# chaiyujin/sdfa-2019

Hardware: AMD Instinct MI355X
Metric: animation frames/s/node (10 s@16 kHz clips); max|Δdgrad| vs CPU ref (higher is better)
Workload: dtype f32

## Files before the change

sdfa-2019_amd/csrc/api_core.cpp:

```cpp
#include "../../include/sdfa_stream.h"
#include "host.h"

#include <climits>
#include <cstdio>
#include <cstring>
#include <string>

static thread_local std::string g_err;

int sdfa_failv(int code, const char *fmt, va_list ap) {
    char buf[512];
    vsnprintf(buf, sizeof buf, fmt, ap);
    g_err = buf;
    return code;
}

int sdfa_fail(int code, const char *fmt, ...) {
    va_list ap;
    va_start(ap, fmt);
    sdfa_failv(code, fmt, ap);
    va_end(ap);
    return code;
}

thread_local int g_sdfa_mel_fft_radix4 = 0;
thread_local int g_sdfa_gather_plain_order = 0;
thread_local int g_sdfa_frontend_two_kernel = 0;
thread_local int g_sdfa_frontend_stream_block = 0;
thread_local int g_sdfa_frontend_stream_slots = 0;
thread_local int g_sdfa_frontend_stream_spin_max = 0;
thread_local int g_sdfa_frontend_stream_phases = 0;
thread_local int g_sdfa_frontend_t_major = 0;
extern thread_local int g_sdfa_gemm_variant;
thread_local int g_sdfa_freq_lstm_shape = 0;
thread_local int g_sdfa_pca_lds = 0;
thread_local int g_sdfa_pca_fp32 = 0;
thread_local int g_sdfa_conv_fp32 = 0;
thread_local int g_sdfa_time_lstm_split = 0;
thread_local int g_sdfa_time_lstm_handoff = 0;
thread_local int g_sdfa_time_lstm_timeout_us = 0;
thread_local int g_sdfa_share_gx0_off = 0;
thread_local int g_sdfa_encoder_dedup_off = 0;
thread_local int g_sdfa_share_hash_bits = 0;
thread_local int g_sdfa_freq_proj_tail = 0;
thread_local int g_sdfa_attn_unfused = 0;

extern "C" {

int sdfa_abi_version(void) { return SDFA_ABI_VERSION; }
int sdfa_stream_abi_version(void) { return SDFA_STREAM_ABI_VERSION; }
const char *sdfa_last_error(void) { return g_err.c_str(); }

int sdfa_debug_set_option(const char *name, int value) {
    struct Option { const char *name; int *var; int lo = INT_MIN, hi = INT_MAX; const char *accepts = nullptr; };
    thread_local const Option options[] = {
        {"attn_unfused", &g_sdfa_attn_unfused},
        {"share_gx0_off", &g_sdfa_share_gx0_off},
        {"encoder_dedup_off", &g_sdfa_encoder_dedup_off},
        {"share_hash_bits", &g_sdfa_share_hash_bits, 0, 32, "0 (the whole hash) or 1..32 low bits"},
        {"freq_proj_tail", &g_sdfa_freq_proj_tail, 0, 2, "0 (rule), 1 (never) or 2 (always)"},
        {"frontend_two_kernel", &g_sdfa_frontend_two_kernel},
        {"frontend_stream_phases", &g_sdfa_frontend_stream_phases},
        {"frontend_stream_spin_max", &g_sdfa_frontend_stream_spin_max, 0, INT_MAX, "0 (default) or a positive poll count"},
        {"frontend_stream_block", &g_sdfa_frontend_stream_block, 0, 256, "0 (default) or 1..256 frames"},
        {"frontend_stream_slots", &g_sdfa_frontend_stream_slots, 0, 256, "0 (default) or 1..256 workgroups per block"},
        {"gather_plain_order", &g_sdfa_gather_plain_order},
        {"mel_fft_radix4", &g_sdfa_mel_fft_radix4},
        {"frontend_t_major", &g_sdfa_frontend_t_major},
        {"time_lstm_timeout_us", &g_sdfa_time_lstm_timeout_us},
        {"time_lstm_handoff", &g_sdfa_time_lstm_handoff},
        {"time_lstm_split", &g_sdfa_time_lstm_split},
        {"gemm_variant", &g_sdfa_gemm_variant},
        {"freq_lstm_shape", &g_sdfa_freq_lstm_shape},
        {"pca_lds", &g_sdfa_pca_lds},
        {"conv_fp32", &g_sdfa_conv_fp32},
        {"pca_fp32", &g_sdfa_pca_fp32},
    };
    for (const Option &o : options)
        if (name && !strcmp(name, o.name)) {
            if (value < o.lo || value > o.hi) return sdfa_fail(SDFA_EINVAL, "%s: %s", o.name, o.accepts);
            *o.var = value;
            return SDFA_OK;
        }
    return sdfa_fail(SDFA_EINVAL, "unknown option '%s'", name ? name : "(null)");
}

}
```

sdfa-2019_amd/csrc/api_forward.cpp:

```cpp
#include "common.h"
#include "host.h"
#include "kernels.h"
#include "model.h"

#include <algorithm>

extern thread_local int g_sdfa_gemm_variant, g_sdfa_freq_lstm_shape, g_sdfa_pca_lds, g_sdfa_pca_fp32, g_sdfa_conv_fp32, g_sdfa_share_gx0_off, g_sdfa_attn_unfused, g_sdfa_encoder_dedup_off,
    g_sdfa_freq_proj_tail, g_sdfa_share_hash_bits;

namespace {

constexpr int64_t CT_WORDS = 2048, CT_FLAGS = 16, ST_WORDS = SDFA_WS_STATUS_BYTES / 4;

struct Ws {
    int64_t P1, X3, HF, Z, GX, H0, H1, KP, QC, QP, ZK, SH, ZU, total;
    int64_t TRUNK, A0, A1, COEF;
    int64_t CT_FREQ, CT_PCA, CT_FLAG;
};

Ws layout(int64_t Nc, bool keep) {
    const int64_t Mc = 64 * Nc;
    Ws w{};
    int64_t o = 0;
    auto take = [&](int64_t n) { int64_t r = o; o += round_up(n, 64); return r; };
// ... 172 lines not shown
                sa.group_key = sa.hash + Mc; sa.group_first = reinterpret_cast<uint32_t *>(sa.group_key + sa.group_slots);
                sa.hash_bits = g_sdfa_share_hash_bits;
                HIP_TRY(sdfa_launch_share_map_content(sa, s));
            }
            pf.end();
            d_ulimit = sa.counts + 1; d_qfull = sa.counts + 2; col_to_u = sa.col_to_u;
            ca.col_src = sa.col_src; ca.col_limit = d_ulimit;
        }
        const int conv_terms = g_sdfa_conv_fp32 ? 0 : stage_terms(m, STAGE_BODY);
        if (m->keep && conv_terms) {
            pf.begin("conv1"); HIP_TRY(sdfa_launch_conv1(ca, s)); pf.end();
            ca.wb = m->cv_wb; ca.terms = conv_terms;
            pf.begin("conv23"); HIP_TRY(sdfa_launch_conv123(ca, s)); pf.end();
        } else if (m->keep) {
            pf.begin("conv1"); HIP_TRY(sdfa_launch_conv1(ca, s)); pf.end();
            pf.begin("conv23"); HIP_TRY(sdfa_launch_conv23(ca, s)); pf.end();
        } else {
            ca.wb = m->cv_wb; ca.terms = conv_terms;
            pf.begin("conv23"); HIP_TRY(sdfa_launch_conv123(ca, s)); pf.end();
        }

        const int fl_terms = stage_terms(m, STAGE_BODY);
        FreqLstmArgs fa{ws + w.X3, m->fl_w, m->fl_b, ws + w.HF, Mc, d_ulimit, m->fl_wb, fl_terms, reinterpret_cast<int *>(ws + w.CT_FREQ),
                        g_sdfa_freq_lstm_shape ? g_sdfa_freq_lstm_shape : (fl_terms ? 0 : m->freq_shape.load()), m->reserved_cus.load()};
        pf.begin("freq_lstm"); HIP_TRY(sdfa_launch_freq_lstm(fa, s)); pf.end();

        GemmArgs g = sdfa_gemm_k4(m->fp_w, 256, ws + w.HF, Mc, ws + w.Z, Mc, 8192);
        g.bias = m->fp_b; g.q_tile_major = 1; g.q_slab_rows = HF_SLAB_ROWS;
        g.terms = stage_terms(m, STAGE_BODY);
        g.reserve_cus = m->reserved_cus.load();
        if (share) { g.D = ws + w.ZU; g.q_limit = split_tail ? d_qfull : d_ulimit; }
        pf.begin("freq_proj");
        HIP_TRY(sdfa_launch_gemm(g, s));
        if (split_tail) {
            GemmTailArgs gt{m->fp_w, ws + w.HF, m->fp_b, ws + w.ZU, Mc, HF_SLAB_ROWS, d_qfull, d_ulimit, (int)fat_grid - 1};
            HIP_TRY(sdfa_launch_gemm_tail(gt, s));
        }
        pf.end();
        const bool share_gx0 = share && !m->keep && stage_terms(m, STAGE_BODY) == 0 && !g_sdfa_share_gx0_off;
        if (share && !share_gx0) {
            pf.begin("share_expand"); HIP_TRY(sdfa_launch_expand_cols(ws + w.ZU, col_to_u, ws + w.Z, 64, Mc, s)); pf.end();
        }

        const float *xin = share_gx0 ? ws + w.ZU : ws + w.Z;
        float *hout[2] = {ws + w.H0, ws + w.H1};
        const char *gxn[2] = {"gx0", "gx1"}, *lsn[2] = {"lstm0", "lstm1"};
        for (int l = 0; l < 2; ++l) {
            const bool mapped = share_gx0 && l == 0;
            float *gx = mapped ? ws + w.HF : ws + w.GX;
            GemmArgs gi = sdfa_gemm_k4(m->gx_w[l], 2048, xin, Mc, gx, Mc, l == 0 ? 256 : 512);
            gi.terms = stage_terms(m, STAGE_BODY);
            gi.reserve_cus = m->reserved_cus.load();
            if (mapped) gi.q_limit = d_ulimit;
            pf.begin(gxn[l]); HIP_TRY(sdfa_launch_gemm(gi, s)); pf.end();
            TimeLstmArgs ta{gx, m->tl_w[l], hout[l], Nc, Mc, m->tl_wb[l], stage_terms(m, STAGE_BODY),
                            reinterpret_cast<unsigned *>(ws + w.CT_FLAG), CT_WORDS - CT_FLAGS, m->tl_w16[l],
                            reinterpret_cast<unsigned *>(ws), m->reserved_cus.load(), mapped ? col_to_u : nullptr};
            pf.begin(lsn[l]); HIP_TRY(sdfa_launch_time_lstm(ta, s)); pf.end();
            xin = hout[l];
        }
        const int at_terms = stage_terms(m, STAGE_ATTENTION);
        const bool key_fused = g_sdfa_attn_unfused != 1;
        pf.begin("attn_proj");
        GemmArgs gk = sdfa_gemm_k4(m->kp_w, 128, ws + w.H1, Mc, ws + w.KP, Mc, 512);
        gk.terms = at_terms;
        if (!key_fused) HIP_TRY(sdfa_launch_gemm(gk, s));
        GemmArgs gc = sdfa_gemm_k4(m->qc_w, 512, ws + w.H1 + 31 * Nc * 4, Mc, ws + w.QC, Nc, 1536);
        gc.seg_k = 512; gc.seg_col = Nc; gc.terms = at_terms;
        HIP_TRY(sdfa_launch_gemm(gc, s));
        GemmArgs gq = sdfa_gemm_k4(m->qp_w, 128, ws + w.QC, Nc, ws + w.QP, Nc, 512);
        gq.terms = at_terms;
        HIP_TRY(sdfa_launch_gemm(gq, s));
        const bool tail_fused = key_fused && (at_terms == 0 || at_terms == 6) && g_sdfa_attn_unfused != 2 && sdfa_attn_fuses_tail(Nc, m->reserved_cus.load());
        if (key_fused) {
            AttnKeyArgs ak{};
            ak.Wk = m->kp_w; ak.H = ws + w.H1; ak.QP = ws + w.QP; ak.v = m->at_v; ak.b = m->at_b;
            ak.S = ws + w.KP;
            ak.Nc = Nc; ak.Mc = Mc; ak.terms = at_terms == 6 ? 0 : at_terms; ak.reserve_cus = m->reserved_cus.load();
            if (tail_fused) {
                ak.fuse_tail = 1; ak.Zk4 = ws + w.ZK; ak.z_out = d_z + f0 * 512; ak.align_out = d_align ? d_align + f0 * 64 : nullptr; ak.N = N;
            }
            HIP_TRY(sdfa_launch_attn_key_score(ak, s));
        }
        pf.end();

        AttnArgs aa{};
        aa.KP = ws + w.KP; aa.QP = ws + w.QP; aa.H = ws + w.H1; aa.v = m->at_v; aa.b = m->at_b;
        aa.Zk4 = ws + w.ZK; aa.z_out = d_z + f0 * 512; aa.align_out = d_align ? d_align + f0 * 64 : nullptr;
        aa.N = N; aa.Nc = Nc; aa.Mc = Mc;
        aa.S = key_fused ? ws + w.KP : nullptr;
        pf.begin("attn"); if (!tail_fused) HIP_TRY(sdfa_launch_attn(aa, s)); pf.end();
    }
    return SDFA_OK;
}

int sdfa_model_autotune(sdfa_model *m, int64_t n_frames, void *d_workspace, int64_t workspace_bytes, void *stream) {
    if (!m || !m->finalized) return sdfa_fail(SDFA_ESTATE, "autotune: model not finalised");
    if (!d_workspace || n_frames <= 0 || ((uintptr_t)d_workspace & 15)) return sdfa_fail(SDFA_EINVAL, "autotune: bad argument");
    const int64_t cap = capacity(workspace_bytes, m->keep);
    if (cap < 128) return sdfa_fail(SDFA_ENOSPACE, "autotune: workspace too small");
    const int64_t Nc = round_up(std::min(cap, n_frames), 128), Mc = 64 * Nc;
    const Ws w = layout(Nc, m->keep);
    float *ws = (float *)d_workspace;
    hipStream_t s = (hipStream_t)stream;
    HIP_TRY(hipMemsetAsync(ws + w.X3, 0, (size_t)2048 * Mc * sizeof(float), s));
    hipEvent_t e0, e1;
    HIP_TRY(hipEventCreate(&e0));
    HIP_TRY(hipEventCreate(&e1));
    static const int forms[] = {9, 8, 5, 3};
    float best_ms = 0.f;
// ... 204 lines not shown
```

sdfa-2019_amd/csrc/api_model.cpp:

```cpp
#include "host.h"
#include "kernels.h"
#include "model.h"

#include <cmath>
#include <cstring>

namespace {

const std::vector<float> *get(const sdfa_model *m, const std::string &name, size_t numel) {
    auto it = m->host.find(name);
    if (it == m->host.end()) { sdfa_fail(SDFA_ESTATE, "tensor '%s' missing", name.c_str()); return nullptr; }
    if (it->second.size() != numel) {
        sdfa_fail(SDFA_ESTATE, "tensor '%s' has %zu elements, expected %zu", name.c_str(), it->second.size(), numel);
        return nullptr;
    }
    return &it->second;
}

struct Packer {
    std::vector<float> buf;
    struct Bind { const float **f; const void **v; size_t o; };
    std::vector<Bind> binds;
    size_t add(size_t n) {
        size_t o = (buf.size() + 63) / 64 * 64;
// ... 244 lines not shown
        const auto perm = gate_perm(128);
        const char *suf[2] = {"", "_reverse"};
        std::vector<float> cat((size_t)512 * 192);
        size_t first = 0;
        std::vector<float> bias(1024);
        auto gate_scale = [](int torch_row) { return torch_row / 128 == 2 ? TWO_LOG2E : LOG2E; };
        for (int d = 0; d < 2; ++d) {
            const std::string k = enc + "6._lstm.";
            auto *wih = get(m, k + "weight_ih_l0" + suf[d], 512 * 64), *whh = get(m, k + "weight_hh_l0" + suf[d], 512 * 128);
            auto *bih = get(m, k + "bias_ih_l0" + suf[d], 512), *bhh = get(m, k + "bias_hh_l0" + suf[d], 512);
            if (!wih || !whh || !bih || !bhh) return SDFA_ESTATE;
            for (int r = 0; r < 512; ++r) {
                const float k = gate_scale(r);
                for (int j = 0; j < 64; ++j) cat[(size_t)r * 192 + j] = (*wih)[(size_t)r * 64 + j] * k;
                for (int j = 0; j < 128; ++j) cat[(size_t)r * 192 + 64 + j] = (*whh)[(size_t)r * 128 + j] * k;
            }
            size_t o = pack_k4(pk, cat.data(), 512, 192, 192, 0, 192, 512, perm.data());
            pack_freq_lstm_bf16(reinterpret_cast<uint16_t *>(&pk.buf[o_flwb]) + (size_t)d * 3 * 24 * 512 * 8, cat.data(), perm.data());
            if (d == 0) first = pk.bind(m->fl_w, o);
            else if (o != first + (size_t)48 * 512 * 4) return sdfa_fail(SDFA_ESTATE, "internal: freq-lstm weights not contiguous");
            for (int p = 0; p < 512; ++p)
                bias[d * 512 + p] = ((*bih)[perm[p]] + (*bhh)[perm[p]]) * gate_scale(perm[p]);
        }
        memcpy(&pk.buf[pk.bind(m->fl_b, pk.add(1024))], bias.data(), 1024 * 4);
    }
    {
        auto *w = get(m, enc + "6._proj.weight", (size_t)256 * 8192), *b = get(m, enc + "6._proj.bias", 256);
        if (!w || !b) return SDFA_ESTATE;
        pk.bind(m->fp_w, pack_k4(pk, w->data(), 256, 8192, 8192, 0, 8192, 256));
        memcpy(&pk.buf[pk.bind(m->fp_b, pk.add(256))], b->data(), 256 * 4);
    }
    {
        size_t o_tlb[2], o_tl16[2];
        const auto perm = gate_perm(256);
        for (int l = 0; l < 2; ++l) o_tlb[l] = pk.bind(m->tl_wb[l], pk.add((size_t)2 * 3 * 32 * 1024 * 8 / 2));
        for (int l = 0; l < 2; ++l) o_tl16[l] = pk.bind(m->tl_w16[l], pk.add((size_t)2 * 16 * 4 * 1024 * 4));
        const char *suf[2] = {"", "_reverse"};
        for (int l = 0; l < 2; ++l) {
            const int Kin = l == 0 ? 256 : 512;
            std::vector<float> both((size_t)2048 * Kin);
            size_t first = 0;
            for (int d = 0; d < 2; ++d) {
                auto *wih = get(m, enc + "9.weight_ih_l" + std::to_string(l) + suf[d], (size_t)1024 * Kin);
                auto *whh = get(m, enc + "9.weight_hh_l" + std::to_string(l) + suf[d], (size_t)1024 * 256);
                if (!wih || !whh) return SDFA_ESTATE;
                for (int p = 0; p < 1024; ++p) memcpy(&both[((size_t)d * 1024 + p) * Kin], &(*wih)[(size_t)perm[p] * Kin], Kin * 4);
                size_t o = pack_k4(pk, whh->data(), 1024, 256, 256, 0, 256, 1024, perm.data());
                pack_rec_bf16(reinterpret_cast<uint16_t *>(&pk.buf[o_tlb[l]]) + (size_t)d * 3 * 32 * 1024 * 8, whh->data(), perm.data());
                pack_rec_16x16x4(&pk.buf[o_tl16[l]] + (size_t)d * 16 * 4 * 1024 * 4, whh->data(), perm.data());
                if (d == 0) first = pk.bind(m->tl_w[l], o);
                else if (o != first + (size_t)64 * 1024 * 4) return sdfa_fail(SDFA_ESTATE, "internal: time-lstm weights not contiguous");
            }
            pk.bind(m->gx_w[l], pack_k4(pk, both.data(), 2048, Kin, Kin, 0, Kin, 2048));
        }
    }
    {
        const std::string k = enc + "10.";
        auto *cq = get(m, k + "_conv_query.weight", (size_t)512 * 512 * 3), *wk = get(m, k + "proj_key.weight", 128 * 512);
        auto *wq = get(m, k + "proj_qry.weight", 128 * 512), *v = get(m, k + "v.weight", 128), *b = get(m, k + "b", 128);
        if (!cq || !wk || !wq || !v || !b) return SDFA_ESTATE;
        pk.bind(m->kp_w, pack_k4(pk, wk->data(), 128, 512, 512, 0, 512, 128));
        pk.bind(m->qp_w, pack_k4(pk, wq->data(), 128, 512, 512, 0, 512, 128));
        std::vector<float> flat((size_t)512 * 1536);
        for (int o = 0; o < 512; ++o)
            for (int c = 0; c < 512; ++c)
                for (int t = 0; t < 3; ++t) flat[(size_t)o * 1536 + t * 512 + c] = (*cq)[((size_t)o * 512 + c) * 3 + t];
        pk.bind(m->qc_w, pack_k4(pk, flat.data(), 512, 1536, 1536, 0, 1536, 512));
        memcpy(&pk.buf[pk.bind(m->at_v, pk.add(128))], v->data(), 512);
        memcpy(&pk.buf[pk.bind(m->at_b, pk.add(128))], b->data(), 512);
    }
    const std::string om = "_output_module.";
    auto pack_basis = [&](int b, const std::vector<float> &compT, int kreal, const std::vector<float> &means) {
        pk.bind(m->pca_q[b], pack_k4(pk, compT.data(), (int)m->pca_cols[b], kreal, kreal, 0, m->pca_K[b], (int)m->pca_ld[b]));
        memcpy(&pk.buf[pk.bind(m->pca_bias[b], pk.add(m->pca_ld[b]))], means.data(), m->pca_cols[b] * 4);
    };
    if (m->head == SDFA_HEAD_DGRAD) {
        if (pack_fc(m, pk, om + "_layers.0", 512, 512, true, ACT_LRELU, m->trunk)) return SDFA_ESTATE;
        const char *brn[2] = {"_scale_layers.", "_rotat_layers."};
        const int nco[2] = {SDFA_COEF_SCALE, SDFA_COEF_ROTAT};
        for (int b = 0; b < 2; ++b) {
            if (pack_fc(m, pk, om + brn[b] + "0", 512, 512, true, ACT_LRELU, m->br[b][0])) return SDFA_ESTATE;
            if (pack_fc(m, pk, om + brn[b] + "1", 256, 512, false, ACT_TANH, m->br[b][1])) return SDFA_ESTATE;
            if (pack_fc(m, pk, om + brn[b] + "2", nco[b], 256, false, ACT_NONE, m->br[b][2])) return SDFA_ESTATE;
        }
        auto *cs = get(m, om + "_scale_pca.compT", (size_t)59856 * 85), *ms = get(m, om + "_scale_pca.means", 59856);
        auto *cr = get(m, om + "_rotat_pca.compT", (size_t)29928 * 180), *mr = get(m, om + "_rotat_pca.means", 29928);
        if (!cs || !ms || !cr || !mr) return SDFA_ESTATE;
        m->pca_n = 2;
        const std::vector<float> *comp[2] = {cs, cr}, *mean[2] = {ms, mr};
        const int kreal[2] = {85, 180};
        for (int b = 0; b < 2; ++b) {
            m->pca_K[b] = b ? 192 : 96; m->pca_k0[b] = b ? 96 : 0; m->pca_group[b] = b ? 3 : 6; m->pca_off[b] = b ? 6 : 0;
            m->pca_cols[b] = b ? 29928 : 59856; m->pca_ld[b] = round_up(m->pca_cols[b], 128);
            pack_basis(b, *comp[b], kreal[b], *mean[b]);
        }
        {
            const int64_t ntb = (m->pca_cols[1] + 95) / 96;
            const size_t o_pqb = pk.bind(m->pca_qb, pk.add((size_t)ntb * 2 * (12 * 192 + 24 * 96) * 8 / 2));
            pack_pca_bf16(reinterpret_cast<uint16_t *>(&pk.buf[o_pqb]), cs->data(), cr->data(), m->pca_cols[0], m->pca_cols[1], ntb);
        }
    } else {
        if (pack_fc(m, pk, om + "_layers.0", 512, 512, true, ACT_LRELU, m->off[0])) return SDFA_ESTATE;
        if (pack_fc(m, pk, om + "_layers.1", 256, 512, false, ACT_TANH, m->off[1])) return SDFA_ESTATE;
        if (pack_fc(m, pk, om + "_layers.2", SDFA_COEF_OFFSETS, 256, false, ACT_NONE, m->off[2])) return SDFA_ESTATE;
        auto *cp = get(m, om + "_pca.compT", (size_t)SDFA_OFFSETS_DIM * 59), *mp = get(m, om + "_pca.means", SDFA_OFFSETS_DIM);
        if (!cp || !mp) return SDFA_ESTATE;
// ... 16 lines not shown
```

sdfa-2019_amd/csrc/kernels.h:

```cpp
#pragma once
#include <hip/hip_runtime.h>
#include <stdint.h>

enum { ACT_NONE = 0, ACT_LRELU = 1, ACT_TANH = 2 };

constexpr int HF_SLAB_ROWS = 2048;
enum { OUT_K4 = 0, OUT_ROW = 1 };
constexpr int SDFA_MAX_DESTS = 8;

struct GemmArgs {
    const float *P;
    const float *Q;
    float *D;
    const float *bias;
    const float *cond_w;
    const int64_t *cond_idx;
    int64_t ldp, ldq, ldd;
    int64_t Ppad, Qpad;
    int64_t Pstore;
    int64_t Qreal;
    int K;
    int seg_k;
    int64_t seg_col;
    int act, out_mode, bias_on_q;
// ... 49 lines not shown
                                  int64_t n_frames, int block, int slots, int producer_consumer, int spin_max, int *status, float *audio_feat, hipStream_t s);
hipError_t sdfa_launch_mel_ring(const FrontendConsts &c, const float *rings, int r, int n_rings, const int64_t *view_ring, const int64_t *view_hi,
                                const int32_t *frame_view, const int64_t *frame_start, const int32_t *prev, const int32_t *shift, int64_t n_frames,
                                int block, int slots, int producer_consumer, int spin_max, int *status, float *audio_feat, hipStream_t s);
hipError_t sdfa_launch_ring_append(float *rings, int r, int n_rings, const int64_t *seg, int n_seg, const float *src, int64_t n_src, hipStream_t s);
hipError_t sdfa_launch_gather_features(const float *mel_table, const int32_t *col_to_u, int64_t n_frames, int64_t Nc, int frame_major,
                                       float *audio_feat, hipStream_t s);

struct ConvArgs {
    const float *audio_feat;
    int64_t N, Nc, Mc;
    const float *w1, *b1, *s1, *t1;
    float *P1;
    const float *w2, *b2, *s2, *t2;
    const float *w3, *b3, *s3, *t3;
    float *X3;
    const int32_t *col_src;
    const int64_t *col_limit;
    const void *wb;
    int terms;
};
hipError_t sdfa_launch_conv1(const ConvArgs &a, hipStream_t s);
hipError_t sdfa_launch_conv23(const ConvArgs &a, hipStream_t s);
hipError_t sdfa_launch_conv123(const ConvArgs &a, hipStream_t s);

struct FreqLstmArgs {
    const float *X3;
    const float *W;
    const float *bias;
    float *HF;
    int64_t Mc;
    const int64_t *col_limit;
    const void *Wb;
    int terms;
    int *tile_counter;
    int shape;
    int reserve_cus;
};
hipError_t sdfa_launch_freq_lstm(const FreqLstmArgs &a, hipStream_t s);

struct TimeLstmArgs {
    const float *GX;
    const float *W;
    float *H;
    int64_t Nc, Mc;
    const void *Wb;
    int terms;
    unsigned *flags;
    int64_t flag_words;
    const float *W16;
    unsigned *status;
    int reserve_cus;
    const int32_t *col_map;
};
hipError_t sdfa_launch_time_lstm(const TimeLstmArgs &a, hipStream_t s);

struct AttnArgs {
    const float *KP;
    const float *QP;
    const float *H;
    const float *v;
    const float *b;
    float *Zk4;
    float *z_out;
    float *align_out;
    int64_t N, Nc, Mc;
    const float *S;
};
hipError_t sdfa_launch_attn(const AttnArgs &a, hipStream_t s);

struct AttnKeyArgs {
    const float *Wk;
    const float *H;
    const float *QP;
    const float *v, *b;
    float *S;
    int64_t Nc, Mc;
    int terms;
    int reserve_cus;
    int ts_shift;
    int fuse_tail;
    float *Zk4, *z_out, *align_out;
    int64_t N;
};
bool sdfa_attn_fuses_tail(int64_t Nc, int reserve_cus);
hipError_t sdfa_launch_attn_key_score(const AttnKeyArgs &a, hipStream_t s);

hipError_t sdfa_launch_rows_to_k4(const float *src, int64_t N, int F, float *dst, int64_t ld, hipStream_t s);
hipError_t sdfa_launch_rows_seg_to_k4(const float *src, int64_t src_ld, int64_t N, int c0, int nf, float *dst, int64_t ld,
                                      int f0, int nf_pad, hipStream_t s);
hipError_t sdfa_launch_k4_to_rows(const float *src, int64_t ld, int64_t N, int F, int f0, int nf, float *dst,
                                  int64_t dst_ld, hipStream_t s);
hipError_t sdfa_launch_tap(const float *src, int what, int64_t N, int64_t Nc, float *dst, hipStream_t s);

struct ShareArgs {
    const int32_t *frame_clip;
    const int64_t *frame_start;
    int hop;
    int t_lo, t_hi;
    int frame_major;
    int64_t N, Nc, Mc;
    int32_t *prev, *shift;
    int32_t *owner, *flag, *uid;
    int32_t *tile_sum;
    int32_t *col_src;
    int32_t *col_to_u;
    int64_t *counts;
    const float *feat;
// ... 103 lines not shown
```

sdfa-2019_amd/csrc/lstm.hip:

```cpp
#include "common.h"
#include "kernels.h"

namespace {

typedef float f32x2 __attribute__((ext_vector_type(2)));
typedef float f32x4n __attribute__((ext_vector_type(4)));

__device__ __forceinline__ f32x2 rcp2(f32x2 d) { return f32x2{__builtin_amdgcn_rcpf(d.x), __builtin_amdgcn_rcpf(d.y)}; }
__device__ __forceinline__ f32x2 exp2n(f32x2 y) { return f32x2{__builtin_amdgcn_exp2f(-y.x), __builtin_amdgcn_exp2f(-y.y)}; }

__device__ __forceinline__ f32x2 sigmoid2(f32x2 x) {
    return rcp2(exp2n(x * 1.4426950408889634f) + 1.0f);
}

__device__ __forceinline__ f32x2 tanh2(f32x2 x) {
    const f32x2 y = x * 2.8853900817779268f;
    const f32x2 e = {__builtin_amdgcn_exp2f(-__builtin_fabsf(y.x)), __builtin_amdgcn_exp2f(-__builtin_fabsf(y.y))};
    const f32x2 t = (1.0f - e) * rcp2(1.0f + e);
    return f32x2{__builtin_copysignf(t.x, x.x), __builtin_copysignf(t.y, x.y)};
}

template <bool FREQ = false>
__device__ __forceinline__ void lstm_cell_quad(const f32x16 &ai, const f32x16 &af, const f32x16 &ag, const f32x16 &ao,
                                               f32x16 &c, int g, float4 &hq) {
// ... 944 lines not shown
            for (int j = 0; j < NT; ++j) ba[j] = brow[j * 32];
#pragma unroll 1
            for (int t = 0; t < 4; ++t) {
                const float4 *bt = brow + t * 16 * BT;
                const float4 *bn = t + 1 < 4 ? bt + 16 * BT : brow;
                const unsigned so = (unsigned)t * (8 * 2048 * 16);
                const unsigned son = t + 1 < 4 ? so + 8 * 2048 * 16 : 0u;
                TL_KB(wa0, wa1, wa2, wa3, ba, wb0, wb1, wb2, wb3, bb, so + 1 * 2048 * 16, bt + 1 * 2 * BT)
                TL_KB(wb0, wb1, wb2, wb3, bb, wa0, wa1, wa2, wa3, ba, so + 2 * 2048 * 16, bt + 2 * 2 * BT)
                TL_KB(wa0, wa1, wa2, wa3, ba, wb0, wb1, wb2, wb3, bb, so + 3 * 2048 * 16, bt + 3 * 2 * BT)
                TL_KB(wb0, wb1, wb2, wb3, bb, wa0, wa1, wa2, wa3, ba, so + 4 * 2048 * 16, bt + 4 * 2 * BT)
                TL_KB(wa0, wa1, wa2, wa3, ba, wb0, wb1, wb2, wb3, bb, so + 5 * 2048 * 16, bt + 5 * 2 * BT)
                TL_KB(wb0, wb1, wb2, wb3, bb, wa0, wa1, wa2, wa3, ba, so + 6 * 2048 * 16, bt + 6 * 2 * BT)
                TL_KB(wa0, wa1, wa2, wa3, ba, wb0, wb1, wb2, wb3, bb, so + 7 * 2048 * 16, bt + 7 * 2 * BT)
                TL_KB(wb0, wb1, wb2, wb3, bb, wa0, wa1, wa2, wa3, ba, son, bn)
            }
            TL_SB()
#undef TL_KB
#undef TL_Q
#undef TL_SB
            wn0 = wa0; wn1 = wa1; wn2 = wa2; wn3 = wa3;
        }
#pragma unroll
        for (int j = 0; j < NT; ++j)
#pragma unroll
            for (int g = 0; g < 4; ++g) {
                float4 hq;
                lstm_cell_quad(acc[0][j], acc[1][j], acc[2][j], acc[3][j], c[j], g, hq);
                const int hq_idx = 8 * wave + 2 * g + h;
                sHn[hq_idx * BT + j * 32 + l31] = hq;
                Hl[(int64_t)(2 * g) * a.Mc + tcol + j * 32] = hq;
                if (s + 1 < 64) {
#pragma unroll
                    for (int gt = 0; gt < 4; ++gt) {
                        const float4 v = TL_GX(tn, gt, g, j);
                        acc[gt][j][4 * g + 0] = v.x; acc[gt][j][4 * g + 1] = v.y; acc[gt][j][4 * g + 2] = v.z; acc[gt][j][4 * g + 3] = v.w;
                    }
                }
            }
        if (MAP && s + 2 < 64) {
            const int t2 = dir ? t - 2 : t + 2;
#pragma unroll
            for (int j = 0; j < NT; ++j) ucol[j] = cmap[(int64_t)t2 * a.Nc + j * 32];
        }
        __syncthreads();
    }
#undef TL_GX
#undef TL_LOAD
#undef TL_W1
}

template <int NT, bool MAP = false>
__global__ __launch_bounds__(512, 2) void time_lstm_kernel(TimeLstmArgs a) { time_lstm_body<NT, MAP>(a); }

template <bool MAP>
__global__ __launch_bounds__(512, 2) void time_lstm_repair_kernel(TimeLstmArgs a, const unsigned *timed_out) {
    if (__hip_atomic_load(timed_out, __ATOMIC_RELAXED, __HIP_MEMORY_SCOPE_AGENT) == 0u) return;
    time_lstm_body<1, MAP>(a);
}

struct SplitCtl {
    unsigned *flags;
    unsigned *timed_out;
    unsigned *status;
    unsigned ticks;
    int mode;
};

__device__ __forceinline__ bool split_wait(const unsigned *pf, unsigned want, const SplitCtl &ctl, int lane) {
    unsigned spins = 0;
    unsigned long long t0 = 0;
    for (;;) {
        const unsigned v = __hip_atomic_load(pf, __ATOMIC_RELAXED, __HIP_MEMORY_SCOPE_AGENT);
        if (__all((int)(v >= want))) return false;
        if ((++spins & 255u) == 0u) {
            const unsigned long long now = __builtin_amdgcn_s_memrealtime();
            if (t0 == 0) t0 = now;
            else if (now - t0 > (unsigned long long)ctl.ticks) {
                if (lane == 0) {
                    __hip_atomic_store(ctl.timed_out, 1u, __ATOMIC_RELAXED, __HIP_MEMORY_SCOPE_AGENT);
                    if (ctl.status) __hip_atomic_fetch_add(ctl.status, 1u, __ATOMIC_RELAXED, __HIP_MEMORY_SCOPE_AGENT);
                }
                return true;
            }
        }
        __builtin_amdgcn_s_sleep(2);
    }
}

template <int G, bool MAP = false>
__global__ __launch_bounds__(512 / G) void time_lstm_split_kernel(TimeLstmArgs a, SplitCtl ctl) {
    unsigned *const flags = ctl.flags;
    const int mode = ctl.mode;
    extern __shared__ float4 sHs[];
    constexpr int BT = 32, NW = 8 / G, NTHR = 64 * NW;
    typedef unsigned int u32x4 __attribute__((ext_vector_type(4)));

    const int tid = threadIdx.x, lane = tid & 63, wave = tid >> 6;
    const int l31 = lane & 31, h = lane >> 5;
    const int q8 = blockIdx.x >> 3;
    const int part = q8 % G, td = (q8 / G) * 8 + (blockIdx.x & 7);
    const int dir = td & 1, hb = part * NW + wave;
    const int64_t n0 = (int64_t)(td >> 1) * BT;

    const float4 *__restrict__ GX = reinterpret_cast<const float4 *>(a.GX);
    f32x16 c;
// ... 568 lines not shown
    {
        hipError_t e = hipFuncSetAttribute(reinterpret_cast<const void *>(time_lstm_bf16_kernel<NT, TERMS>),
                                           hipFuncAttributeMaxDynamicSharedMemorySize, (int)lds);
        if (e != hipSuccess) return e;
    }
    hipLaunchKernelGGL((time_lstm_bf16_kernel<NT, TERMS>), dim3((unsigned)(a.Nc / (32 * NT) * 2)), dim3(512), lds, s, a);
    return hipGetLastError();
}

extern thread_local int g_sdfa_time_lstm_handoff;
extern thread_local int g_sdfa_time_lstm_timeout_us;

template <bool MAP>
static hipError_t launch_time_repair(const TimeLstmArgs &a, hipStream_t s) {
    const size_t lds = 2 * 64 * 32 * sizeof(float4);
    hipError_t e = hipFuncSetAttribute(reinterpret_cast<const void *>(time_lstm_repair_kernel<MAP>), hipFuncAttributeMaxDynamicSharedMemorySize, (int)lds);
    if (e != hipSuccess) return e;
    hipLaunchKernelGGL(time_lstm_repair_kernel<MAP>, dim3((unsigned)(a.Nc / 32 * 2)), dim3(512), lds, s, a, a.flags);
    return hipGetLastError();
}

static SplitCtl split_ctl(const TimeLstmArgs &a) {
    const long long us = g_sdfa_time_lstm_timeout_us > 0 ? g_sdfa_time_lstm_timeout_us : 20000;
    return SplitCtl{a.flags + 4, a.flags, a.status, (unsigned)std::min<long long>(us * 100, 0xffffffffll), g_sdfa_time_lstm_handoff};
}

template <int G, bool MAP>
static hipError_t launch_time_split(const TimeLstmArgs &a, hipStream_t s) {
    const size_t lds = 96 * 1024;
    hipError_t e = hipFuncSetAttribute(reinterpret_cast<const void *>(time_lstm_split_kernel<G, MAP>), hipFuncAttributeMaxDynamicSharedMemorySize, (int)lds);
    if (e != hipSuccess) return e;
    const unsigned grid = (unsigned)(a.Nc / 32 * 2 * G);
    e = hipMemsetAsync(a.flags, 0, ((size_t)grid + 4) * sizeof(unsigned), s);
    if (e != hipSuccess) return e;
    hipLaunchKernelGGL((time_lstm_split_kernel<G, MAP>), dim3(grid), dim3(512 / G), lds, s, a, split_ctl(a));
    e = hipGetLastError();
    return e != hipSuccess ? e : launch_time_repair<MAP>(a, s);
}

template <bool MAP>
static hipError_t launch_time_split16(const TimeLstmArgs &a, hipStream_t s) {
    const size_t lds = 96 * 1024;
    hipError_t e = hipFuncSetAttribute(reinterpret_cast<const void *>(time_lstm_split16_kernel<MAP>), hipFuncAttributeMaxDynamicSharedMemorySize, (int)lds);
    if (e != hipSuccess) return e;
    const unsigned grid = (unsigned)(a.Nc / 16 * 2 * 2);
    e = hipMemsetAsync(a.flags, 0, ((size_t)grid + 4) * sizeof(unsigned), s);
    if (e != hipSuccess) return e;
    hipLaunchKernelGGL(time_lstm_split16_kernel<MAP>, dim3(grid), dim3(256), lds, s, a, split_ctl(a));
    e = hipGetLastError();
    return e != hipSuccess ? e : launch_time_repair<MAP>(a, s);
}

extern thread_local int g_sdfa_time_lstm_split;

template <bool MAP>
static hipError_t launch_time_any(const TimeLstmArgs &a, hipStream_t s) {
    const bool big = (a.Nc / 64) * 2 >= 256;
    if (!a.terms && a.flags && g_sdfa_time_lstm_split != 1) {
        int dev = 0, cus = 256;
        if (hipGetDevice(&dev) != hipSuccess || hipDeviceGetAttribute(&cus, hipDeviceAttributeMultiprocessorCount, dev) != hipSuccess) cus = 256;
        cus -= a.reserve_cus;
        const int64_t wg1 = a.Nc / 32 * 2;
        const bool range_ok = (int64_t)64 * a.Mc * 16 + (int64_t)a.Mc * 16 < 0x7fffffff && a.Nc % 128 == 0 && a.flag_words >= wg1 * 2 + 4;
        const int G = (range_ok && wg1 * 2 <= cus) ? 2 : 0;
        if (range_ok && a.W16 && g_sdfa_time_lstm_split != 32 && wg1 * 4 <= cus && a.flag_words >= wg1 * 4 + 4) return launch_time_split16<MAP>(a, s);
        if (g_sdfa_time_lstm_split == 16) return hipErrorInvalidValue;
        if (G == 2) return launch_time_split<2, MAP>(a, s);
    }
    if (a.terms) {
        if (!a.Wb || MAP) return hipErrorInvalidValue;
        if (a.terms == 6) return launch_time_bf16<1, 6>(a, s);
        if (a.terms == 1) return big ? launch_time_bf16<2, 1>(a, s) : launch_time_bf16<1, 1>(a, s);
        return big ? launch_time_bf16<2, 3>(a, s) : launch_time_bf16<1, 3>(a, s);
    }
    return big ? launch_time<2, MAP>(a, s) : launch_time<1, MAP>(a, s);
}

hipError_t sdfa_launch_time_lstm(const TimeLstmArgs &a, hipStream_t s) {
    return a.col_map ? launch_time_any<true>(a, s) : launch_time_any<false>(a, s);
}
```

sdfa-2019_amd/csrc/model.h:

```cpp
#pragma once
#include "../../include/sdfa_hip.h"

#include <hip/hip_runtime.h>
#include <atomic>
#include <map>
#include <mutex>
#include <string>
#include <vector>

struct sdfa_model {
    int head = SDFA_HEAD_DGRAD;
    bool finalized = false;
    bool keep = false;
    bool profile = false;
    std::map<std::string, std::vector<float>> host;
    void *blob = nullptr;
    const float *w1, *b1, *s1, *t1, *w2, *b2, *s2, *t2, *w3, *b3, *s3, *t3;
    const float *fl_w, *fl_b, *fp_w, *fp_b;
    const void *fl_wb = nullptr;
    const void *cv_wb = nullptr;
    int precision = SDFA_PREC_FP32;
    const float *gx_w[2], *tl_w[2];
    const void *tl_wb[2] = {nullptr, nullptr};
    const float *tl_w16[2] = {nullptr, nullptr};
    const float *kp_w, *qc_w, *qp_w, *at_v, *at_b;
    struct Fc { const float *w, *b, *cw; int K, P, Ppad, Pstore; int act; };
    Fc trunk, br[2][3], off[3];
    int pca_n = 0;
    const float *pca_q[2], *pca_bias[2];
    const void *pca_qb = nullptr;
    int pca_K[2], pca_k0[2], pca_group[2], pca_off[2];
    std::atomic<int> freq_shape{9};
    std::atomic<int> reserved_cus{0};
    int64_t pca_ld[2], pca_cols[2];
    int64_t out_dim, coef_dim;
    struct Ev { std::string stage; hipEvent_t a, b; };
    mutable std::vector<Ev> events;
    mutable std::mutex ev_mu;
};
```

Before: 148,600.

## Fuse layer-1 input projection into time-LSTM recurrence kernel

Adds a time-LSTM kernel for layer 1 that computes the input-to-gate projection (X·Wx) inside the recurrent loop, using a combined packed Wx|Wh weight image streamed through buffer loads. X tiles are double-buffered through LDS. This removes the separate gx GEMM launch and the round trip of its gate output through global memory. A selection rule enables it only when the split kernels are not chosen and the workgroup count fills the CUs well; otherwise the old path runs. The cost is extra recurrent-loop work per step and extra model memory for the packed weights.

```diff
diff --git a/sdfa-2019_amd/csrc/api_core.cpp b/sdfa-2019_amd/csrc/api_core.cpp
--- a/sdfa-2019_amd/csrc/api_core.cpp
+++ b/sdfa-2019_amd/csrc/api_core.cpp
@@ -37,6 +37,7 @@
 thread_local int g_sdfa_pca_fp32 = 0;
 thread_local int g_sdfa_conv_fp32 = 0;
 thread_local int g_sdfa_time_lstm_split = 0;
+thread_local int g_sdfa_time_lstm_fuse_x = 0;
 thread_local int g_sdfa_time_lstm_handoff = 0;
 thread_local int g_sdfa_time_lstm_timeout_us = 0;
 thread_local int g_sdfa_share_gx0_off = 0;
@@ -70,6 +71,7 @@
         {"time_lstm_timeout_us", &g_sdfa_time_lstm_timeout_us},
         {"time_lstm_handoff", &g_sdfa_time_lstm_handoff},
         {"time_lstm_split", &g_sdfa_time_lstm_split},
+        {"time_lstm_fuse_x", &g_sdfa_time_lstm_fuse_x, 0, 3, "0 (rule), 1 (never), 2 or 3 (always, 32- / 64-frame tiles)"},
         {"gemm_variant", &g_sdfa_gemm_variant},
         {"freq_lstm_shape", &g_sdfa_freq_lstm_shape},
         {"pca_lds", &g_sdfa_pca_lds},
diff --git a/sdfa-2019_amd/csrc/api_forward.cpp b/sdfa-2019_amd/csrc/api_forward.cpp
--- a/sdfa-2019_amd/csrc/api_forward.cpp
+++ b/sdfa-2019_amd/csrc/api_forward.cpp
@@ -248,10 +248,13 @@
             gi.terms = stage_terms(m, STAGE_BODY);
             gi.reserve_cus = m->reserved_cus.load();
             if (mapped) gi.q_limit = d_ulimit;
-            pf.begin(gxn[l]); HIP_TRY(sdfa_launch_gemm(gi, s)); pf.end();
             TimeLstmArgs ta{gx, m->tl_w[l], hout[l], Nc, Mc, m->tl_wb[l], stage_terms(m, STAGE_BODY),
                             reinterpret_cast<unsigned *>(ws + w.CT_FLAG), CT_WORDS - CT_FLAGS, m->tl_w16[l],
                             reinterpret_cast<unsigned *>(ws), m->reserved_cus.load(), mapped ? col_to_u : nullptr};
+            if (l == 1 && !m->keep) { ta.X = xin; ta.Wxh = m->tl_wxh1; }
+            pf.begin(gxn[l]);
+            if (!sdfa_time_lstm_fuses_x(ta)) HIP_TRY(sdfa_launch_gemm(gi, s));
+            pf.end();
             pf.begin(lsn[l]); HIP_TRY(sdfa_launch_time_lstm(ta, s)); pf.end();
             xin = hout[l];
         }
diff --git a/sdfa-2019_amd/csrc/api_model.cpp b/sdfa-2019_amd/csrc/api_model.cpp
--- a/sdfa-2019_amd/csrc/api_model.cpp
+++ b/sdfa-2019_amd/csrc/api_model.cpp
@@ -320,6 +320,17 @@
                 else if (o != first + (size_t)64 * 1024 * 4) return sdfa_fail(SDFA_ESTATE, "internal: time-lstm weights not contiguous");
             }
             pk.bind(m->gx_w[l], pack_k4(pk, both.data(), 2048, Kin, Kin, 0, Kin, 2048));
+            if (l == 1) {
+                const size_t o_x = pk.bind(m->tl_wxh1, pk.add((size_t)2 * 192 * 1024 * 4));
+                for (int d = 0; d < 2; ++d) {
+                    auto *whh = get(m, enc + "9.weight_hh_l1" + suf[d], (size_t)1024 * 256);
+                    float *img = &pk.buf[o_x + (size_t)d * 192 * 1024 * 4];
+                    for (int p = 0; p < 1024; ++p) {
+                        for (int k = 0; k < 512; ++k) img[((size_t)(k / 4) * 1024 + p) * 4 + k % 4] = both[((size_t)d * 1024 + p) * 512 + k];
+                        for (int k = 0; k < 256; ++k) img[((size_t)(128 + k / 4) * 1024 + p) * 4 + k % 4] = (*whh)[(size_t)perm[p] * 256 + k];
+                    }
+                }
+            }
         }
     }
     {
diff --git a/sdfa-2019_amd/csrc/kernels.h b/sdfa-2019_amd/csrc/kernels.h
--- a/sdfa-2019_amd/csrc/kernels.h
+++ b/sdfa-2019_amd/csrc/kernels.h
@@ -125,8 +125,11 @@
     unsigned *status;
     int reserve_cus;
     const int32_t *col_map;
+    const float *X = nullptr;
+    const float *Wxh = nullptr;
 };
 hipError_t sdfa_launch_time_lstm(const TimeLstmArgs &a, hipStream_t s);
+int sdfa_time_lstm_fuses_x(const TimeLstmArgs &a);
 
 struct AttnArgs {
     const float *KP;
diff --git a/sdfa-2019_amd/csrc/lstm.hip b/sdfa-2019_amd/csrc/lstm.hip
--- a/sdfa-2019_amd/csrc/lstm.hip
+++ b/sdfa-2019_amd/csrc/lstm.hip
@@ -1020,6 +1020,157 @@
 
 template <int NT, bool MAP = false>
 __global__ __launch_bounds__(512, 2) void time_lstm_kernel(TimeLstmArgs a) { time_lstm_body<NT, MAP>(a); }
+
+template <int NT>
+__global__ __launch_bounds__(512, 2) void time_lstm_fused_kernel(TimeLstmArgs a) {
+    extern __shared__ float4 sHt[];
+    constexpr int BT = 32 * NT;
+
+    const int tid = threadIdx.x, lane = tid & 63, wave = tid >> 6;
+    const int l31 = lane & 31, h = lane >> 5;
+    const int dir = blockIdx.x & 1;
+    const int64_t n0 = (int64_t)(blockIdx.x >> 1) * BT;
+
+    float4 *__restrict__ H = reinterpret_cast<float4 *>(a.H);
+    float4 *const sX = sHt + 2 * 64 * BT;
+
+    f32x16 c[NT];
+#pragma unroll
+    for (int j = 0; j < NT; ++j)
+#pragma unroll
+        for (int r = 0; r < 16; ++r) c[j][r] = 0.f;
+
+    const float4 *__restrict__ Xl = reinterpret_cast<const float4 *>(a.X) + (int64_t)(2 * wave + (NT == 1 ? h : 0)) * a.Mc + n0 + (NT == 1 ? l31 : lane);
+    float4 *const xw = sX + 2 * wave * BT + lane;
+    float4 xr0, xr1;
+#define TF_XLOAD(t_, sl)                                                                                         \
+    {                                                                                                            \
+        const float4 *xs = Xl + (int64_t)((sl) * 16) * a.Mc + (int64_t)(t_) * a.Nc;                              \
+        xr0 = xs[0];                                                                                             \
+        if (NT > 1) xr1 = xs[a.Mc];                                                                              \
+    }
+#define TF_XSTORE(buf)                                                                                           \
+    {                                                                                                            \
+        xw[(buf) * 16 * BT] = xr0;                                                                               \
+        if (NT > 1) xw[(buf) * 16 * BT + 64] = xr1;                                                              \
+    }
+    float4 *__restrict__ Hl = H + (int64_t)(dir * 64 + wave * 8 + h) * a.Mc + n0 + l31;
+
+    typedef unsigned int u32x4 __attribute__((ext_vector_type(4)));
+    const unsigned long long wptr = (unsigned long long)(reinterpret_cast<const float4 *>(a.Wxh) + (size_t)dir * 192 * 1024 + wave * 128);
+    const unsigned long long wuni = ((unsigned long long)(unsigned)__builtin_amdgcn_readfirstlane((int)(wptr >> 32)) << 32) |
+                                    (unsigned long long)(unsigned)__builtin_amdgcn_readfirstlane((int)(unsigned)wptr);
+    const __amdgpu_buffer_rsrc_t wrs = __builtin_amdgcn_make_buffer_rsrc((void *)wuni, 0, (192 * 1024 - 7 * 128) * 16, 0x00020000);
+    const unsigned woff = (unsigned)((l31 + h * 1024) * 16);
+#define TF_W1(so, g_) __builtin_bit_cast(float4, (u32x4)__builtin_amdgcn_raw_buffer_load_b128(wrs, woff + 512 * (g_), so, 0))
+    constexpr unsigned KB = 2048 * 16;
+    float4 wn0, wn1, wn2, wn3;
+    TF_XLOAD(dir ? 63 : 0, 0)
+    wn0 = TF_W1(0u, 0); wn1 = TF_W1(0u, 1); wn2 = TF_W1(0u, 2); wn3 = TF_W1(0u, 3);
+    TF_XSTORE(0)
+    __syncthreads();
+
+#define TF_SB() __builtin_amdgcn_sched_barrier(0);
+#define TF_Q(W0, W1, W2, W3, B, q)                                                                               \
+    _Pragma("unroll") for (int j = 0; j < NT; ++j) acc[0][j] = MFMA(f4c(W0, q), f4c(B[j], q), acc[0][j]);        \
+    _Pragma("unroll") for (int j = 0; j < NT; ++j) acc[1][j] = MFMA(f4c(W1, q), f4c(B[j], q), acc[1][j]);        \
+    _Pragma("unroll") for (int j = 0; j < NT; ++j) acc[2][j] = MFMA(f4c(W2, q), f4c(B[j], q), acc[2][j]);        \
+    _Pragma("unroll") for (int j = 0; j < NT; ++j) acc[3][j] = MFMA(f4c(W3, q), f4c(B[j], q), acc[3][j]);
+#define TF_QZ(W0, W1, W2, W3, B, q)                                                                              \
+    _Pragma("unroll") for (int j = 0; j < NT; ++j) acc[0][j] = MFMA(f4c(W0, q), f4c(B[j], q), zero16);           \
+    _Pragma("unroll") for (int j = 0; j < NT; ++j) acc[1][j] = MFMA(f4c(W1, q), f4c(B[j], q), zero16);           \
+    _Pragma("unroll") for (int j = 0; j < NT; ++j) acc[2][j] = MFMA(f4c(W2, q), f4c(B[j], q), zero16);           \
+    _Pragma("unroll") for (int j = 0; j < NT; ++j) acc[3][j] = MFMA(f4c(W3, q), f4c(B[j], q), zero16);
+#define TF_KB_(Q0, AFTER_W, AT_B, CW0, CW1, CW2, CW3, CB, NW0, NW1, NW2, NW3, NB, so, bp)                        \
+    {                                                                                                            \
+        TF_SB() NW0 = TF_W1(so, 0); NW1 = TF_W1(so, 1); TF_SB()                                                  \
+        Q0(CW0, CW1, CW2, CW3, CB, 0)                                                                            \
+        TF_SB() NW2 = TF_W1(so, 2); NW3 = TF_W1(so, 3); AFTER_W TF_SB()                                          \
+        TF_Q(CW0, CW1, CW2, CW3, CB, 1)                                                                          \
+        TF_SB() AT_B NB[0] = (bp)[0]; TF_SB()                                                                    \
+        TF_Q(CW0, CW1, CW2, CW3, CB, 2)                                                                          \
+        TF_SB() if (NT > 1) NB[NT - 1] = (bp)[32 * (NT - 1)]; TF_SB()                                            \
+        TF_Q(CW0, CW1, CW2, CW3, CB, 3)                                                                          \
+    }
+#define TF_NONE
+#define TF_KB(...) TF_KB_(TF_Q, TF_NONE, TF_NONE, __VA_ARGS__)
+#define TF_HANDOVER asm volatile("s_waitcnt lgkmcnt(0)\n\ts_barrier" ::: "memory");
+#define TF_XTRIP(Q0, i_)                                                                                                          \
+    {                                                                                                                             \
+        const int nb = ((i_) & 1) ^ 1;                                                                                            \
+        const float4 *bt = xrow + ((i_) & 1) * 16 * BT;                                                                           \
+        const float4 *bn = (i_) < 7 ? xrow + nb * 16 * BT : hrow;                                                                 \
+        const unsigned so = (unsigned)(i_) * (8 * KB);                                                                            \
+        const unsigned son = ((i_) < 7 || s > 0) ? so + 8 * KB : 0u;        \
+        const int tl = (i_) < 7 ? t : tn, sl = (i_) < 7 ? (i_) + 1 : 0;                                                           \
+        TF_KB_(Q0, TF_XLOAD(tl, sl), TF_NONE, wa0, wa1, wa2, wa3, ba, wb0, wb1, wb2, wb3, bb, so + 1 * KB, bt + 1 * 2 * BT)      \
+        TF_KB(wb0, wb1, wb2, wb3, bb, wa0, wa1, wa2, wa3, ba, so + 2 * KB, bt + 2 * 2 * BT)                                       \
+        TF_KB(wa0, wa1, wa2, wa3, ba, wb0, wb1, wb2, wb3, bb, so + 3 * KB, bt + 3 * 2 * BT)                                       \
+        TF_KB_(TF_Q, TF_NONE, TF_XSTORE(nb), wb0, wb1, wb2, wb3, bb, wa0, wa1, wa2, wa3, ba, so + 4 * KB, bt + 4 * 2 * BT)        \
+        TF_KB(wa0, wa1, wa2, wa3, ba, wb0, wb1, wb2, wb3, bb, so + 5 * KB, bt + 5 * 2 * BT)                                       \
+        TF_KB(wb0, wb1, wb2, wb3, bb, wa0, wa1, wa2, wa3, ba, so + 6 * KB, bt + 6 * 2 * BT)                                       \
+        TF_KB(wa0, wa1, wa2, wa3, ba, wb0, wb1, wb2, wb3, bb, so + 7 * KB, bt + 7 * 2 * BT)                                       \
+        TF_KB_(TF_Q, TF_NONE, TF_HANDOVER, wb0, wb1, wb2, wb3, bb, wa0, wa1, wa2, wa3, ba, son, bn)                               \
+    }
+    const f32x16 zero16 = {0.f, 0.f, 0.f, 0.f, 0.f, 0.f, 0.f, 0.f, 0.f, 0.f, 0.f, 0.f, 0.f, 0.f, 0.f, 0.f};
+    const float4 *const xrow = sX + h * BT + l31;
+    for (int s = 0; s < 64; ++s) {
+        const int t = dir ? 63 - s : s;
+        const int tn = s + 1 < 64 ? (dir ? t - 1 : t + 1) : t;
+        const int64_t tcol = (int64_t)t * a.Nc;
+        const float4 *hrow = sHt + (size_t)(s & 1) * 64 * BT + h * BT + l31;
+        float4 *sHn = sHt + (size_t)((s & 1) ^ 1) * 64 * BT;
+
+        f32x16 acc[4][NT];
+        float4 wa0 = wn0, wa1 = wn1, wa2 = wn2, wa3 = wn3, wb0, wb1, wb2, wb3, ba[NT], bb[NT];
+#pragma unroll
+        for (int j = 0; j < NT; ++j) ba[j] = xrow[j * 32];
+        TF_XTRIP(TF_QZ, 0)
+#pragma unroll 1
+        for (int i = 1; i < 8; ++i) TF_XTRIP(TF_Q, i)
+        if (s > 0) {
+#pragma unroll 1
+            for (int tr = 0; tr < 4; ++tr) {
+                const float4 *bt = hrow + tr * 16 * BT;
+                const float4 *bn = tr + 1 < 4 ? bt + 16 * BT : xrow;
+                const unsigned so = (unsigned)(8 + tr) * (8 * KB);
+                const unsigned son = tr + 1 < 4 ? so + 8 * KB : 0u;
+                TF_KB(wa0, wa1, wa2, wa3, ba, wb0, wb1, wb2, wb3, bb, so + 1 * KB, bt + 1 * 2 * BT)
+                TF_KB(wb0, wb1, wb2, wb3, bb, wa0, wa1, wa2, wa3, ba, so + 2 * KB, bt + 2 * 2 * BT)
+                TF_KB(wa0, wa1, wa2, wa3, ba, wb0, wb1, wb2, wb3, bb, so + 3 * KB, bt + 3 * 2 * BT)
+                TF_KB(wb0, wb1, wb2, wb3, bb, wa0, wa1, wa2, wa3, ba, so + 4 * KB, bt + 4 * 2 * BT)
+                TF_KB(wa0, wa1, wa2, wa3, ba, wb0, wb1, wb2, wb3, bb, so + 5 * KB, bt + 5 * 2 * BT)
+                TF_KB(wb0, wb1, wb2, wb3, bb, wa0, wa1, wa2, wa3, ba, so + 6 * KB, bt + 6 * 2 * BT)
+                TF_KB(wa0, wa1, wa2, wa3, ba, wb0, wb1, wb2, wb3, bb, so + 7 * KB, bt + 7 * 2 * BT)
+                TF_KB(wb0, wb1, wb2, wb3, bb, wa0, wa1, wa2, wa3, ba, son, bn)
+            }
+        }
+        TF_SB()
+        wn0 = wa0; wn1 = wa1; wn2 = wa2; wn3 = wa3;
+#pragma unroll
+        for (int j = 0; j < NT; ++j)
+#pragma unroll
+            for (int g = 0; g < 4; ++g) {
+                float4 hq;
+                lstm_cell_quad(acc[0][j], acc[1][j], acc[2][j], acc[3][j], c[j], g, hq);
+                const int hq_idx = 8 * wave + 2 * g + h;
+                sHn[hq_idx * BT + j * 32 + l31] = hq;
+                Hl[(int64_t)(2 * g) * a.Mc + tcol + j * 32] = hq;
+            }
+        __syncthreads();
+    }
+#undef TF_XTRIP
+#undef TF_HANDOVER
+#undef TF_KB
+#undef TF_NONE
+#undef TF_KB_
+#undef TF_QZ
+#undef TF_Q
+#undef TF_SB
+#undef TF_W1
+#undef TF_XSTORE
+#undef TF_XLOAD
+}
 
 template <bool MAP>
 __global__ __launch_bounds__(512, 2) void time_lstm_repair_kernel(TimeLstmArgs a, const unsigned *timed_out) {
@@ -1694,21 +1845,43 @@
 }
 
 extern thread_local int g_sdfa_time_lstm_split;
+extern thread_local int g_sdfa_time_lstm_fuse_x;
+
+static bool time_big(const TimeLstmArgs &a) { return (a.Nc / 64) * 2 >= 256; }
+
+static int time_split_form(const TimeLstmArgs &a) {
+    if (a.terms || !a.flags || g_sdfa_time_lstm_split == 1) return 0;
+    int dev = 0, cus = 256;
+    if (hipGetDevice(&dev) != hipSuccess || hipDeviceGetAttribute(&cus, hipDeviceAttributeMultiprocessorCount, dev) != hipSuccess) cus = 256;
+    cus -= a.reserve_cus;
+    const int64_t wg1 = a.Nc / 32 * 2;
+    const bool range_ok = (int64_t)64 * a.Mc * 16 + (int64_t)a.Mc * 16 < 0x7fffffff && a.Nc % 128 == 0 && a.flag_words >= wg1 * 2 + 4;
+    if (range_ok && a.W16 && g_sdfa_time_lstm_split != 32 && wg1 * 4 <= cus && a.flag_words >= wg1 * 4 + 4) return 16;
+    if (g_sdfa_time_lstm_split == 16) return -1;
+    return (range_ok && wg1 * 2 <= cus) ? 2 : 0;
+}
+
+template <int NT>
+static hipError_t launch_time_fused(const TimeLstmArgs &a, hipStream_t s) {
+    if (a.Nc % (32 * NT)) return hipErrorInvalidValue;
+    const size_t lds = (2 * 64 + 2 * 16) * 32 * NT * sizeof(float4);
+    hipError_t e = hipFuncSetAttribute(reinterpret_cast<const void *>(time_lstm_fused_kernel<NT>), hipFuncAttributeMaxDynamicSharedMemorySize, (int)lds);
+    if (e != hipSuccess) return e;
+    hipLaunchKernelGGL((time_lstm_fused_kernel<NT>), dim3((unsigned)(a.Nc / (32 * NT) * 2)), dim3(512), lds, s, a);
+    return hipGetLastError();
+}
 
 template <bool MAP>
 static hipError_t launch_time_any(const TimeLstmArgs &a, hipStream_t s) {
-    const bool big = (a.Nc / 64) * 2 >= 256;
-    if (!a.terms && a.flags && g_sdfa_time_lstm_split != 1) {
-        int dev = 0, cus = 256;
-        if (hipGetDevice(&dev) != hipSuccess || hipDeviceGetAttribute(&cus, hipDeviceAttributeMultiprocessorCount, dev) != hipSuccess) cus = 256;
-        cus -= a.reserve_cus;
-        const int64_t wg1 = a.Nc / 32 * 2;
-        const bool range_ok = (int64_t)64 * a.Mc * 16 + (int64_t)a.Mc * 16 < 0x7fffffff && a.Nc % 128 == 0 && a.flag_words >= wg1 * 2 + 4;
-        const int G = (range_ok && wg1 * 2 <= cus) ? 2 : 0;
-        if (range_ok && a.W16 && g_sdfa_time_lstm_split != 32 && wg1 * 4 <= cus && a.flag_words >= wg1 * 4 + 4) return launch_time_split16<MAP>(a, s);
-        if (g_sdfa_time_lstm_split == 16) return hipErrorInvalidValue;
-        if (G == 2) return launch_time_split<2, MAP>(a, s);
-    }
+    const bool big = time_big(a);
+    if (!MAP) {
+        const int nt = sdfa_time_lstm_fuses_x(a);
+        if (nt) return nt == 2 ? launch_time_fused<2>(a, s) : launch_time_fused<1>(a, s);
+    }
+    const int split = time_split_form(a);
+    if (split == 16) return launch_time_split16<MAP>(a, s);
+    if (split < 0) return hipErrorInvalidValue;
+    if (split == 2) return launch_time_split<2, MAP>(a, s);
     if (a.terms) {
         if (!a.Wb || MAP) return hipErrorInvalidValue;
         if (a.terms == 6) return launch_time_bf16<1, 6>(a, s);
@@ -1718,6 +1891,17 @@
     return big ? launch_time<2, MAP>(a, s) : launch_time<1, MAP>(a, s);
 }
 
+int sdfa_time_lstm_fuses_x(const TimeLstmArgs &a) {
+    if (!a.X || !a.Wxh || a.terms || a.col_map || g_sdfa_time_lstm_fuse_x == 1) return 0;
+    if (g_sdfa_time_lstm_fuse_x == 2) return 1;
+    if (g_sdfa_time_lstm_fuse_x == 3) return 2;
+    if (time_split_form(a) != 0) return 0;
+    const int nt = time_big(a) ? 2 : 1;
+    const int64_t wgs = a.Nc / (32 * nt) * 2, cus = std::max(1, sdfa_cu_count());
+    const int64_t rounds = (wgs + cus - 1) / cus;
+    return wgs * 100 >= rounds * cus * 93 ? nt : 0;
+}
+
 hipError_t sdfa_launch_time_lstm(const TimeLstmArgs &a, hipStream_t s) {
     return a.col_map ? launch_time_any<true>(a, s) : launch_time_any<false>(a, s);
 }
diff --git a/sdfa-2019_amd/csrc/model.h b/sdfa-2019_amd/csrc/model.h
--- a/sdfa-2019_amd/csrc/model.h
+++ b/sdfa-2019_amd/csrc/model.h
@@ -23,6 +23,7 @@
     const float *gx_w[2], *tl_w[2];
     const void *tl_wb[2] = {nullptr, nullptr};
     const float *tl_w16[2] = {nullptr, nullptr};
+    const float *tl_wxh1 = nullptr;
     const float *kp_w, *qc_w, *qp_w, *at_v, *at_b;
     struct Fc { const float *w, *b, *cw; int K, P, Ppad, Pstore; int act; };
     Fc trunk, br[2][3], off[3];
```

Result: faster. 151,100, median of 6 (+1.7%).
